# wq2012/SpectralCluster

Hardware: AMD Instinct MI355X
Metric: predict() calls/sec, n=8192 d=256 ICASSP2018 (GraphCut, eigengap k in [2,20], cosine k-means) (higher is better)
Workload: dtype f64; 1 GPU; icassp2018_graphcut_n8192_d256_k8_max20; n_samples=8192, n_features=256, parallelism=replicas x1, collectives=none

## Files before the change

### spectralcluster_amd/csrc/eig.hip

```cpp
#include <algorithm>
#include <cstring>
#include <mutex>

#include "sc_internal.h"

namespace sc {

typedef double v4f64 __attribute__((ext_vector_type(4)));
constexpr int B = kEigBlock;
constexpr int RB = 256 / B;
static_assert(B == 8 || B == 16, "block width must divide the 16-wide MFMA tile");

__device__ __forceinline__ uint64_t splitmix64(uint64_t x) {
  x += 0x9E3779B97F4A7C15ull;
  x = (x ^ (x >> 30)) * 0xBF58476D1CE4E5B9ull;
  x = (x ^ (x >> 27)) * 0x94D049BB133111EBull;
  return x ^ (x >> 31);
}
__device__ __forceinline__ double hash_uniform(uint64_t seed, uint64_t idx) {
  const uint64_t h = splitmix64(seed ^ splitmix64(idx));
  return (double)(h >> 11) * (2.0 / 9007199254740992.0) - 1.0;
}

__global__ void k_random_block(double* W, int n, uint64_t seed) {
  const int e = blockIdx.x * blockDim.x + threadIdx.x;
  if (e < n * B) W[e] = hash_uniform(seed, (uint64_t)e);
}

__global__ void k_refill_deficient(double* W, int n, const int* flags,
                                   uint64_t seed) {
  const int e = blockIdx.x * blockDim.x + threadIdx.x;
  if (e >= n * B) return;
  if ((flags[0] >> (e & (B - 1))) & 1) W[e] = hash_uniform(seed, (uint64_t)e);
}

constexpr int kMvWaves = 8;
__device__ __forceinline__ void block_matvec_body(
    const double* __restrict__ S, int ld, int n, const double* __restrict__ cvec,
    const double* __restrict__ pvec, const double* __restrict__ V, int ldv,
    const double* __restrict__ Vs, double* __restrict__ W) {
  __shared__ double red[kMvWaves][64][4];
  const int lane = threadIdx.x & 63;
  const int wave = threadIdx.x >> 6;
  const int li = lane & 15, lg = lane >> 4;
  const int r0 = blockIdx.x * 16;
  int ri = r0 + li;
  ri = ri < n ? ri : n - 1;
  const double* srow = S + (size_t)ri * ld + 2 * lg;
  v4f64 acc0 = {0.0, 0.0, 0.0, 0.0}, acc1 = {0.0, 0.0, 0.0, 0.0};
  const int nchunks = (n + 31) / 32;
  double2 cur[4], nxt[4];
  auto load = [&](double2* dst, int ch) {
    const int kb = ch * 32 + 2 * lg;
#pragma unroll
    for (int q = 0; q < 4; ++q) {
      if (kb + 8 * q + 1 < ld)
        dst[q] = *reinterpret_cast<const double2*>(srow + ch * 32 + 8 * q);
      else
        dst[q] = make_double2(0.0, 0.0);
    }
  };
  int ch = wave;
  if (ch < nchunks) load(cur, ch);
  for (; ch < nchunks; ch += kMvWaves) {
    if (ch + kMvWaves < nchunks) load(nxt, ch + kMvWaves);
    const int kb = ch * 32 + 2 * lg;
    double b[8];
#pragma unroll
    for (int t = 0; t < 8; ++t) {
      const int k = kb + 8 * (t >> 1) + (t & 1);
      b[t] = (k < n && li < B) ? Vs[(size_t)k * B + li] : 0.0;
    }
#pragma unroll
    for (int q = 0; q < 4; ++q) {
      const double a0 = (kb + 8 * q < n) ? cur[q].x : 0.0;
      const double a1 = (kb + 8 * q + 1 < n) ? cur[q].y : 0.0;
      acc0 = __builtin_amdgcn_mfma_f64_16x16x4f64(a0, b[2 * q], acc0, 0, 0, 0);
      acc1 = __builtin_amdgcn_mfma_f64_16x16x4f64(a1, b[2 * q + 1], acc1, 0, 0, 0);
    }
#pragma unroll
    for (int q = 0; q < 4; ++q) cur[q] = nxt[q];
  }
#pragma unroll
  for (int r = 0; r < 4; ++r) red[wave][lane][r] = acc0[r] + acc1[r];
  __syncthreads();
  if (wave == 0) {
#pragma unroll
    for (int r = 0; r < 4; ++r) {
      double sum = 0.0;
#pragma unroll
      for (int w = 0; w < kMvWaves; ++w) sum += red[w][lane][r];
      const int row = r0 + lg + 4 * r;
      if (row < n && li < B)
        W[(size_t)row * B + li] =
            __builtin_fma(cvec ? cvec[row] : 1.0, sum,
                          pvec ? pvec[row] * V[(size_t)row * ldv + li] : 0.0);
    }
  }
}
__global__ __launch_bounds__(64 * kMvWaves) void k_block_matvec(
    const double* __restrict__ S, int ld, int n, const double* __restrict__ cvec,
    const double* __restrict__ pvec, const double* __restrict__ V, int ldv,
    const double* __restrict__ Vs, double* __restrict__ W) {
  block_matvec_body(S, ld, n, cvec, pvec, V, ldv, Vs, W);
}
__global__ __launch_bounds__(64 * kMvWaves) void k_block_matvec_g(const GroupOf<MatvecItem> g) {
  const MatvecItem& a = g.s[blockIdx.y];
  if ((int)blockIdx.x * 16 >= a.n) return;
  block_matvec_body(a.S, a.ld, a.n, a.cvec, a.pvec, a.V, a.ldv, a.Vs, a.W);
}

constexpr int kSymTile = 128;
constexpr int kSymPitch = 34;
__device__ __forceinline__ int sym_item_id(int I, int J, int nt) {
  return I * nt - I * (I - 1) / 2 + (J - I);
}
__device__ __forceinline__ void block_matvec_sym_body(
    const double* __restrict__ S, int ld, int n, const double* __restrict__ Vs,
    double* __restrict__ pdirect, double* __restrict__ pmirror, int nt) {
  __shared__ __attribute__((aligned(16))) double smem[4 * 32 * kSymPitch];
  int I = 0, rem = blockIdx.x, rowlen = nt;
  while (rem >= rowlen) {
    rem -= rowlen;
    --rowlen;
    ++I;
  }
  const int J = I + rem;
  const bool diag = I == J;
  const int lane = threadIdx.x & 63, wave = threadIdx.x >> 6;
  const int li = lane & 15, lg = lane >> 4;
  const int r0 = I * kSymTile + 32 * wave;
  const int c0 = J * kSymTile;
  double* patch = smem + wave * (32 * kSymPitch);
  double bm[8];
#pragma unroll
  for (int t = 0; t < 8; ++t) {
    const int row = r0 + 4 * t + lg;
    bm[t] = (row < n && li < B) ? Vs[(size_t)row * B + li] : 0.0;
  }
  v4f64 accd[2] = {{0.0, 0.0, 0.0, 0.0}, {0.0, 0.0, 0.0, 0.0}};
  v4f64 accm[4][2];
#pragma unroll
  for (int cs = 0; cs < 4; ++cs)
#pragma unroll
    for (int ct = 0; ct < 2; ++ct) accm[cs][ct] = (v4f64){0.0, 0.0, 0.0, 0.0};
  double2 a[1][2][4];
  auto load = [&](int buf, int cs) {
#pragma unroll
    for (int rt = 0; rt < 2; ++rt) {
      int row = r0 + 16 * rt + li;
      row = row < n ? row : n - 1;
      const double* src = S + (size_t)row * ld + c0 + 32 * cs + 2 * lg;
#pragma unroll
      for (int q = 0; q < 4; ++q) {
        if (c0 + 32 * cs + 8 * q + 2 * lg + 1 < ld)
          a[buf][rt][q] = *reinterpret_cast<const double2*>(src + 8 * q);
        else
          a[buf][rt][q] = make_double2(0.0, 0.0);
      }
    }
  };
#pragma unroll
  for (int cs = 0; cs < 4; ++cs) {
    constexpr int cur = 0;
    load(cur, cs);
    const int kb = c0 + 32 * cs + 2 * lg;
#pragma unroll
    for (int rt = 0; rt < 2; ++rt) {
      const bool rok = r0 + 16 * rt + li < n;
#pragma unroll
      for (int q = 0; q < 4; ++q) {
        if (!rok || kb + 8 * q >= n) a[cur][rt][q].x = 0.0;
        if (!rok || kb + 8 * q + 1 >= n) a[cur][rt][q].y = 0.0;
      }
    }
    double b[8];
#pragma unroll
    for (int t = 0; t < 8; ++t) {
      const int k = kb + 8 * (t >> 1) + (t & 1);
      b[t] = (k < n && li < B) ? Vs[(size_t)k * B + li] : 0.0;
    }
#pragma unroll
    for (int rt = 0; rt < 2; ++rt)
#pragma unroll
      for (int q = 0; q < 4; ++q) {
        accd[rt] = __builtin_amdgcn_mfma_f64_16x16x4f64(a[cur][rt][q].x, b[2 * q], accd[rt], 0, 0, 0);
        accd[rt] = __builtin_amdgcn_mfma_f64_16x16x4f64(a[cur][rt][q].y, b[2 * q + 1], accd[rt], 0, 0, 0);
      }
    if (!diag) {
#pragma unroll
      for (int rt = 0; rt < 2; ++rt)
#pragma unroll
        for (int q = 0; q < 4; ++q)
          *reinterpret_cast<double2*>(patch + (16 * rt + li) * kSymPitch + 8 * q + 2 * lg) =
              a[cur][rt][q];
      __builtin_amdgcn_fence(__ATOMIC_RELEASE, "wavefront");
      __builtin_amdgcn_wave_barrier();
#pragma unroll
      for (int ct = 0; ct < 2; ++ct)
#pragma unroll
        for (int t = 0; t < 8; ++t) {
          const double at = patch[(4 * t + lg) * kSymPitch + 16 * ct + li];
          accm[cs][ct] = __builtin_amdgcn_mfma_f64_16x16x4f64(at, bm[t], accm[cs][ct], 0, 0, 0);
        }
      __builtin_amdgcn_fence(__ATOMIC_ACQUIRE, "wavefront");
      __builtin_amdgcn_wave_barrier();
    }
  }
  const size_t item = blockIdx.x;
  if (li < B) {
#pragma unroll
    for (int rt = 0; rt < 2; ++rt)
#pragma unroll
      for (int r = 0; r < 4; ++r)
        pdirect[(item * kSymTile + 32 * wave + 16 * rt + lg + 4 * r) * B + li] = accd[rt][r];
  }
  if (diag) return;
  __syncthreads();
  double* red = smem;
  if (li < B) {
#pragma unroll
    for (int cs = 0; cs < 4; ++cs)
#pragma unroll
      for (int ct = 0; ct < 2; ++ct)
#pragma unroll
        for (int r = 0; r < 4; ++r)
          red[(wave * kSymTile + 32 * cs + 16 * ct + lg + 4 * r) * B + li] = accm[cs][ct][r];
  }
  __syncthreads();
  for (int e = threadIdx.x; e < kSymTile * B; e += 256)
    pmirror[item * (kSymTile * B) + e] =
        ((red[e] + red[kSymTile * B + e]) + red[2 * kSymTile * B + e]) + red[3 * kSymTile * B + e];
}
__global__ __launch_bounds__(256) void k_block_matvec_sym(
    const double* __restrict__ S, int ld, int n, const double* __restrict__ Vs,
    double* __restrict__ pdirect, double* __restrict__ pmirror, int nt) {
  block_matvec_sym_body(S, ld, n, Vs, pdirect, pmirror, nt);
}
__global__ __launch_bounds__(256) void k_block_matvec_sym_g(const GroupOf<MatvecItem> g) {
  const MatvecItem& a = g.s[blockIdx.y];
  const int nt = (a.n + kSymTile - 1) / kSymTile;
  if ((int)blockIdx.x >= nt * (nt + 1) / 2) return;
  block_matvec_sym_body(a.S, a.ld, a.n, a.Vs, a.slabs, a.slabs + (size_t)(nt * (nt + 1) / 2) * kSymTile * B, nt);
}

__device__ __forceinline__ void matvec_sym_reduce_body(
    const double* __restrict__ pdirect, const double* __restrict__ pmirror, int nt, int n,
    const double* __restrict__ cvec, const double* __restrict__ pvec,
    const double* __restrict__ V, int ldv, double* __restrict__ W) {
  const int R = blockIdx.x / 4;
  const int e = (blockIdx.x & 3) * 256 + threadIdx.x;
  const int rl = e / B, v = e % B;
  const int row = R * kSymTile + rl;
  double acc = 0.0;
  const int total = nt;
  for (int s0 = 0; s0 < total; s0 += 8) {
    double x[8];
#pragma unroll
    for (int u = 0; u < 8; ++u) {
      const int sidx = s0 + u;
      x[u] = 0.0;
      if (sidx < nt - R) {
        x[u] = pdirect[(size_t)sym_item_id(R, R + sidx, nt) * (kSymTile * B) + e];
      } else if (sidx < total) {
        x[u] = pmirror[(size_t)sym_item_id(sidx - (nt - R), R, nt) * (kSymTile * B) + e];
      }
    }
#pragma unroll
    for (int u = 0; u < 8; ++u) acc += x[u];
  }
  if (row < n) W[(size_t)row * B + v] =
      __builtin_fma(cvec ? cvec[row] : 1.0, acc, pvec ? pvec[row] * V[(size_t)row * ldv + v] : 0.0);
}
__global__ __launch_bounds__(256) void k_matvec_sym_reduce(
    const double* __restrict__ pdirect, const double* __restrict__ pmirror, int nt, int n,
    const double* __restrict__ cvec, const double* __restrict__ pvec,
    const double* __restrict__ V, int ldv, double* __restrict__ W) {
  matvec_sym_reduce_body(pdirect, pmirror, nt, n, cvec, pvec, V, ldv, W);
}
__global__ __launch_bounds__(256) void k_matvec_sym_reduce_g(const GroupOf<MatvecItem> g) {
  const MatvecItem& a = g.s[blockIdx.y];
  const int nt = (a.n + kSymTile - 1) / kSymTile;
  if ((int)blockIdx.x >= nt * 4) return;
  matvec_sym_reduce_body(a.slabs, a.slabs + (size_t)(nt * (nt + 1) / 2) * kSymTile * B, nt, a.n,
                         a.cvec, a.pvec, a.V, a.ldv, a.W);
}

constexpr int kProjGroups = 256 / B;
constexpr int kProjAcc = (kLdq + kProjGroups - 1) / kProjGroups;
__global__ __launch_bounds__(256) void k_proj_partial(
    const double* __restrict__ Q, int ldq, int m, const double* __restrict__ W,
    int n, double* __restrict__ partial) {
  __shared__ double Ql[8][kLdq];
  __shared__ double Wl[8][B];
  const int tid = threadIdx.x;
  const int jj = tid % B, ig = tid / B;
  const int rows_per = (n + gridDim.x - 1) / gridDim.x;
  const int rbeg = blockIdx.x * rows_per;
  const int rend = min(n, rbeg + rows_per);
  double acc[kProjAcc];
#pragma unroll
  for (int q = 0; q < kProjAcc; ++q) acc[q] = 0.0;
  for (int r = rbeg; r < rend; r += 8) {
    __syncthreads();
    for (int e = tid; e < 8 * m; e += 256) {
      const int rr = e / m, i = e - rr * m;
      Ql[rr][i] = (r + rr < rend) ? Q[(size_t)(r + rr) * ldq + i] : 0.0;
    }
    if (tid < 8 * B) {
      const int rr = tid / B;
      Wl[rr][jj] = (r + rr < rend) ? W[(size_t)(r + rr) * B + jj] : 0.0;
    }
    __syncthreads();
#pragma unroll
    for (int rr = 0; rr < 8; ++rr) {
      const double w = Wl[rr][jj];
#pragma unroll
      for (int q = 0; q < kProjAcc; ++q)
        if (ig + kProjGroups * q < m)
          acc[q] = __builtin_fma(Ql[rr][ig + kProjGroups * q], w, acc[q]);
    }
  }
  double* out = partial + (size_t)blockIdx.x * (kLdq * B);
#pragma unroll
  for (int q = 0; q < kProjAcc; ++q)
    if (ig + kProjGroups * q < m) out[(ig + kProjGroups * q) * B + jj] = acc[q];
}

__global__ __launch_bounds__(256) void k_reduce_H(
    const double* __restrict__ partial, int nparts, int m, double* __restrict__ Hbuf,
    double* __restrict__ T, int ldt, int col0, int accumulate,
    double* __restrict__ hsq) {
  __shared__ double sq[32];
  const int tid = threadIdx.x;
  const int sub = tid & 7;
  const int e = blockIdx.x * 32 + (tid >> 3);
  double h = 0.0;
  if (e < m * B)
    for (int g = sub; g < nparts; g += 8) h += partial[(size_t)g * (kLdq * B) + e];
  h += __shfl_xor(h, 1);
  h += __shfl_xor(h, 2);
  h += __shfl_xor(h, 4);
  if (sub == 0) {
    if (e < m * B) {
      Hbuf[e] = h;
      if (T != nullptr) {
        const int i = e / B, j = col0 + (e % B);
        if (i <= j) {
          const double v = accumulate ? T[(size_t)i * ldt + j] + h : h;
          T[(size_t)i * ldt + j] = v;
          T[(size_t)j * ldt + i] = v;
        }
      }
    } else {
      h = 0.0;
    }
    sq[tid >> 3] = h * h;
  }
  __syncthreads();
  if (tid < B) {
    double s = 0.0;
    for (int q = tid; q < 32; q += B) s += sq[q];
    atomicAdd(&hsq[tid], s);
  }
}

__global__ __launch_bounds__(256) void k_update_block(
    const double* __restrict__ Q, int ldq, int m, const double* __restrict__ Hbuf,
    double* __restrict__ W, int n) {
  __shared__ double Hl[kLdq * B];
  __shared__ double Ql[RB][kLdq + 1];
  const int tid = threadIdx.x;
  const int jj = tid % B, rr = tid / B;
  const int r0 = blockIdx.x * RB;
  for (int e = tid; e < m * B; e += 256) Hl[e] = Hbuf[e];
  for (int e = tid; e < RB * m; e += 256) {
    const int a = e / m, i = e - a * m;
    Ql[a][i] = (r0 + a < n) ? Q[(size_t)(r0 + a) * ldq + i] : 0.0;
  }
  __syncthreads();
  const int r = r0 + rr;
  if (r < n) {
    double acc = W[(size_t)r * B + jj];
    for (int i = 0; i < m; ++i) acc = __builtin_fma(-Ql[rr][i], Hl[i * B + jj], acc);
    W[(size_t)r * B + jj] = acc;
  }
}

__device__ __forceinline__ void chol8_wave(const double* G, double* __restrict__ Rinv,
                                           const double* __restrict__ hsq,
                                           int* __restrict__ flags,
                                           int* __restrict__ defect_flag, int flag_mode,
                                           int* __restrict__ sticky_flag = nullptr,
                                           int sticky_m = 0, bool sticky_on_defect = true);

__global__ __launch_bounds__(256) void k_reduce_chol(
    const double* __restrict__ partial, int nparts, double* __restrict__ Rinv,
    double* __restrict__ Gsave, const double* __restrict__ hsq,
    int* __restrict__ flags, int* __restrict__ defect_flag, int flag_mode) {
  static_assert(B == 8, "the factorisation below maps the 8 x 8 matrix onto one wavefront");
  __shared__ double G[B * B];
  const int tid = threadIdx.x;
  {
    constexpr int kLanes = 256 / (B * B);
    const int e = tid / kLanes, sub = tid % kLanes;
    double g = 0.0;
    for (int q = sub; q < nparts; q += kLanes) g += partial[(size_t)q * (kLdq * B) + e];
#pragma unroll
    for (int o = 1; o < kLanes; o <<= 1) g += __shfl_xor(g, o);
    if (sub == 0) {
      G[e] = g;
      if (Gsave) Gsave[e] = g;
    }
  }
  __syncthreads();
  if (tid >= 64) return;
  chol8_wave(G, Rinv, hsq, flags, defect_flag, flag_mode);
}

__device__ __forceinline__ void chol8_wave(const double* G, double* __restrict__ Rinv,
                                           const double* __restrict__ hsq,
                                           int* __restrict__ flags,
                                           int* __restrict__ defect_flag, int flag_mode,
                                           int* __restrict__ sticky_flag, int sticky_m,
                                           bool sticky_on_defect) {
// ... 962 lines not shown
```

### spectralcluster_amd/csrc/kmeans_chain.hip

```cpp
#include <algorithm>
#include <cstring>
#include <mutex>

#include "kmeans_common.h"
#include "sc_internal.h"

namespace sc {

constexpr int kKmT = 128;
constexpr int kKmW = kKmT / 64;
constexpr int kKmMaxG = 1024;

struct KmChain {
  const double* ET;
  int lde, n, k, G;
  const double* rnd;
  int trials, first_center, max_iter;
  double* closest;
  double* xsq;
  long long* labels64;
  double* centroids_out;
  double* pm;
  double* meang;
  double* ppot;
  double* pT;
  double* pS[2];
  double* pD[2];
  double* meand;
  double* cent[2];
  int* seeds;
  int* cand[2];
  int* info;
};

__device__ __forceinline__ double km_ordered_sum(const double* src, int stride, int G) {
  double acc = 0.0;
  for (int g0 = 0; g0 < G; g0 += 16) {
    double v[16];
#pragma unroll
    for (int u = 0; u < 16; ++u) v[u] = (g0 + u < G) ? src[(size_t)(g0 + u) * stride] : 0.0;
#pragma unroll
    for (int u = 0; u < 16; ++u) acc += v[u];
  }
  return acc;
}

__device__ __forceinline__ void km_mean(const KmChain& a, double* mean) {
  if ((int)threadIdx.x < a.k) mean[threadIdx.x] = a.meang[threadIdx.x];
}

__device__ __forceinline__ void km_meanreduce_body(const KmChain& a) {
  if ((int)threadIdx.x < a.k)
    a.meang[threadIdx.x] = km_ordered_sum(a.pm + threadIdx.x, 64, a.G) / (double)a.n;
}
__global__ __launch_bounds__(64) void km_meanreduce(const KmChain a) { km_meanreduce_body(a); }
__global__ __launch_bounds__(64) void km_meanreduce_g(const GroupOf<KmChain> g) {
  const KmChain& a = g.s[blockIdx.y];
  if (a.G > 0) km_meanreduce_body(a);
}

template <int KC>
__device__ __forceinline__ void km_load_row(const KmChain& a, int r, double (&v)[KC]) {
#pragma unroll
  for (int j = 0; j < KC; ++j) v[j] = (j < a.k && r < a.n) ? a.ET[(size_t)j * a.lde + r] : 0.0;
}

template <int KC>
__device__ __forceinline__ void km_colsum_body(const KmChain& a) {
  __shared__ double sm[kKmW][KC];
  const int tid = threadIdx.x, r = blockIdx.x * kKmT + tid;
  double v[KC];
  km_load_row<KC>(a, r, v);
#pragma unroll
  for (int j = 0; j < KC; ++j) {
    const double s = wave_sum(v[j]);
    if ((tid & 63) == 0) sm[tid >> 6][j] = s;
  }
  __syncthreads();
  if (tid < a.k) {
    double t = 0.0;
#pragma unroll
    for (int w = 0; w < kKmW; ++w) t += sm[w][tid];
    a.pm[(size_t)blockIdx.x * 64 + tid] = t;
  }
}
template <int KC>
__global__ __launch_bounds__(kKmT) void km_colsum(const KmChain a) {
  km_colsum_body<KC>(a);
}
template <int KC>
__global__ __launch_bounds__(kKmT) void km_colsum_g(const GroupOf<KmChain> g) {
  const KmChain& a = g.s[blockIdx.y];
  if ((int)blockIdx.x >= a.G) return;
  km_colsum_body<KC>(a);
}

template <int KC>
__device__ __forceinline__ double km_dist(const double (&v)[KC], const double* mean,
                                          const double* crow, double csq, double xsq, int k) {
  double dot = 0.0;
#pragma unroll
  for (int j = 0; j < KC; ++j)
    if (j < k) dot += crow[j] * (v[j] - mean[j]);
  double d = -2.0 * dot;
  d += csq;
  d += xsq;
  return fmax(d, 0.0);
}

template <int KC>
__device__ __forceinline__ void km_first_body(const KmChain& a) {
  __shared__ double mean[KC], crow[KC], sm[kKmW];
  __shared__ double csq;
  const int tid = threadIdx.x, r = blockIdx.x * kKmT + tid;
  km_mean(a, mean);
  double v[KC];
  km_load_row<KC>(a, r, v);
  __syncthreads();
  if (tid < a.k) crow[tid] = a.ET[(size_t)tid * a.lde + a.first_center] - mean[tid];
  __syncthreads();
  if (tid == 0) {
    double s2 = 0.0;
    for (int j = 0; j < a.k; ++j) s2 += crow[j] * crow[j];
    csq = s2;
  }
  double xs = 0.0;
#pragma unroll
  for (int j = 0; j < KC; ++j)
    if (j < a.k) {
      const double x = v[j] - mean[j];
      xs += x * x;
    }
  __syncthreads();
  double d = 0.0;
  if (r < a.n) {
    d = km_dist<KC>(v, mean, crow, csq, xs, a.k);
    a.xsq[r] = xs;
    a.closest[r] = d;
  }
  const double tot = block_sum<kKmW>(d, sm);
  if (tid == 0) a.ppot[blockIdx.x] = tot;
  if (blockIdx.x == 0) {
    if (tid == 0) {
      a.seeds[0] = a.first_center;
      a.info[0] = 0;
      a.info[8] = 0;
    }
    if (tid < 8) a.cand[1][tid] = a.n - 1;
  }
}
template <int KC>
__global__ __launch_bounds__(kKmT) void km_first(const KmChain a) {
  km_first_body<KC>(a);
}
template <int KC>
__global__ __launch_bounds__(kKmT) void km_first_g(const GroupOf<KmChain> g) {
  const KmChain& a = g.s[blockIdx.y];
  if ((int)blockIdx.x >= a.G) return;
  km_first_body<KC>(a);
}

__device__ __forceinline__ int km_best_trial(const KmChain& a, double* pots) {
  if ((int)threadIdx.x < a.trials) pots[threadIdx.x] = km_ordered_sum(a.pT + threadIdx.x, 8, a.G);
  __syncthreads();
  int best = 0;
  double bp = pots[0];
  for (int t = 1; t < a.trials; ++t)
    if (pots[t] < bp) {
      bp = pots[t];
      best = t;
    }
  return best;
}

__device__ __forceinline__ void km_prefix(const double* src, int stride, int G, double* part,
                                          double* offset, double* total) {
  for (int g = threadIdx.x; g < G; g += kKmT) part[g] = src[(size_t)g * stride];
  __syncthreads();
  if (threadIdx.x == 0) {
    double off = 0.0, tot = 0.0;
    for (int g = 0; g < G; ++g) {
      if (g == (int)blockIdx.x) off = tot;
      tot += part[g];
    }
    part[kKmMaxG] = off;
    part[kKmMaxG + 1] = tot;
  }
  __syncthreads();
  *offset = part[kKmMaxG];
  *total = part[kKmMaxG + 1];
}

template <int KC>
__device__ __forceinline__ void km_select_body(const KmChain& a, int c) {
  __shared__ double mean[KC], crow[KC], sm[kKmW], pots[8], rvals[8], scan[kKmT];
  __shared__ double part[kKmMaxG + 2];
  __shared__ double csq;
  const int tid = threadIdx.x, lane = tid & 63, wave = tid >> 6;
  const int r = blockIdx.x * kKmT + tid;
  double cl = r < a.n ? a.closest[r] : 0.0;
  double offset = 0.0, pot = 0.0;
  if (c >= 2) {
    km_mean(a, mean);
    double v[KC];
    km_load_row<KC>(a, r, v);
    const double xs = r < a.n ? a.xsq[r] : 0.0;
    __syncthreads();
    const int best = km_best_trial(a, pots);
    const int row = a.cand[(c - 1) & 1][best];
    if (tid < a.k) crow[tid] = a.ET[(size_t)tid * a.lde + row] - mean[tid];
    __syncthreads();
    if (tid == 0) {
      double s2 = 0.0;
      for (int j = 0; j < a.k; ++j) s2 += crow[j] * crow[j];
      csq = s2;
      if (blockIdx.x == 0) a.seeds[c - 1] = row;
    }
    __syncthreads();
    if (r < a.n) {
      cl = fmin(cl, km_dist<KC>(v, mean, crow, csq, xs, a.k));
      a.closest[r] = cl;
    }
    km_prefix(a.pT + best, 8, a.G, part, &offset, &pot);
  } else {
    km_prefix(a.ppot, 1, a.G, part, &offset, &pot);
  }
  if (tid < a.trials) rvals[tid] = a.rnd[(c - 1) * a.trials + tid] * pot;
  double v = cl;
#pragma unroll
  for (int o = 1; o < 64; o <<= 1) {
    const double u = __shfl_up(v, o);
    if (lane >= o) v += u;
  }
  __syncthreads();
  if (lane == 63) sm[wave] = v;
  __syncthreads();
  double woff = 0.0;
  for (int w = 0; w < wave; ++w) woff += sm[w];
  scan[tid] = v + woff;
  __syncthreads();
  if (r < a.n) {
    const double incl = offset + scan[tid];
    const double excl = tid == 0 ? offset : offset + scan[tid - 1];
    for (int t = 0; t < a.trials; ++t) {
      const double rv = rvals[t];
      if ((rv > excl || r == 0) && rv <= incl) atomicMin(&a.cand[c & 1][t], r);
    }
  }
}
template <int KC>
__global__ __launch_bounds__(kKmT) void km_select(const KmChain a, int c) {
  km_select_body<KC>(a, c);
}
template <int KC>
__global__ __launch_bounds__(kKmT) void km_select_g(const GroupOf<KmChain> g, int c) {
  const KmChain& a = g.s[blockIdx.y];
  if ((int)blockIdx.x >= a.G || c >= a.k) return;
  km_select_body<KC>(a, c);
}

template <int KC>
__device__ __forceinline__ void km_trials_body(const KmChain& a, int c) {
  __shared__ double mean[KC], crow[8][KC], csq[8], sm[kKmW];
  const int tid = threadIdx.x, r = blockIdx.x * kKmT + tid;
  km_mean(a, mean);
  double v[KC];
  km_load_row<KC>(a, r, v);
  const double xs = r < a.n ? a.xsq[r] : 0.0;
  const double cl = r < a.n ? a.closest[r] : 0.0;
  __syncthreads();
  for (int e = tid; e < a.trials * a.k; e += kKmT) {
    const int t = e / a.k, j = e - t * a.k;
    crow[t][j] = a.ET[(size_t)j * a.lde + a.cand[c & 1][t]] - mean[j];
  }
  __syncthreads();
  if (tid < a.trials) {
    double s2 = 0.0;
    for (int j = 0; j < a.k; ++j) s2 += crow[tid][j] * crow[tid][j];
    csq[tid] = s2;
  }
  __syncthreads();
  for (int t = 0; t < a.trials; ++t) {
    double d = 0.0;
    if (r < a.n) d = fmin(cl, km_dist<KC>(v, mean, crow[t], csq[t], xs, a.k));
    const double tot = block_sum<kKmW>(d, sm);
    if (tid == 0) a.pT[(size_t)blockIdx.x * 8 + t] = tot;
  }
  if (blockIdx.x == 0 && tid < 8) a.cand[(c + 1) & 1][tid] = a.n - 1;
}
template <int KC>
__global__ __launch_bounds__(kKmT) void km_trials(const KmChain a, int c) {
  km_trials_body<KC>(a, c);
}
template <int KC>
__global__ __launch_bounds__(kKmT) void km_trials_g(const GroupOf<KmChain> g, int c) {
  const KmChain& a = g.s[blockIdx.y];
  if ((int)blockIdx.x >= a.G || c >= a.k) return;
  km_trials_body<KC>(a, c);
}

template <int KC>
__device__ __forceinline__ void km_cluster_partials(const KmChain& a, const double (&v)[KC],
                                                    const double* shift, int label, int r,
                                                    double* vals, int* labs, double* out) {
  const int tid = threadIdx.x, k = a.k;
  labs[tid] = r < a.n ? label : -1;
#pragma unroll
  for (int j = 0; j < KC; ++j)
    if (j < k) vals[tid * KC + j] = v[j] - shift[j];
  __syncthreads();
  const int r0 = blockIdx.x * kKmT;
  const int nsum = k * k + 2 * k;
  for (int base = 0; base < nsum; base += kKmT / 4) {
    const int e = base + (tid >> 2), seg = tid & 3;
    double acc = 0.0;
    if (e < nsum) {
      const int t0 = seg * (kKmT / 4);
      if (e < k * k) {
        const int c2 = e / k, j = e - c2 * k;
#pragma unroll 8
        for (int t = t0; t < t0 + kKmT / 4; ++t) acc += labs[t] == c2 ? vals[t * KC + j] : 0.0;
      } else if (e < k * k + k) {
        const int c2 = e - k * k;
#pragma unroll 8
        for (int t = t0; t < t0 + kKmT / 4; ++t) acc += labs[t] == c2 ? 1.0 : 0.0;
      } else {
        const int c2 = e - k * k - k;
#pragma unroll 8
        for (int t = t0; t < t0 + kKmT / 4; ++t)
          acc += (labs[t] == c2 && r0 + t > 0) ? 1.0 : 0.0;
      }
    }
    const double a1 = __shfl_down(acc, 1), a2 = __shfl_down(acc, 2), a3 = __shfl_down(acc, 3);
    if (e < nsum && seg == 0) out[e] = ((acc + a1) + a2) + a3;
  }
}

template <int KC>
__device__ __forceinline__ void km_lloyd_body(const KmChain& a) {
  extern __shared__ __attribute__((aligned(16))) double dyn[];
  double* vals = dyn;
  int* labs = reinterpret_cast<int*>(vals + kKmT * KC);
  __shared__ double mean[KC], cent[KC * KC], cnorm[KC], pots[8];
  __shared__ int seeds[KC];
  const int tid = threadIdx.x, r = blockIdx.x * kKmT + tid, k = a.k;
  km_mean(a, mean);
  double v[KC];
  km_load_row<KC>(a, r, v);
  __syncthreads();
  if (k > 1) {
    const int best = km_best_trial(a, pots);
    if (tid == 0) {
      seeds[k - 1] = a.cand[(k - 1) & 1][best];
      if (blockIdx.x == 0) a.seeds[k - 1] = seeds[k - 1];
    }
  }
  if (tid < k - 1 || (k == 1 && tid == 0)) seeds[tid] = a.seeds[tid];
  __syncthreads();
  for (int e = tid; e < k * k; e += kKmT) {
    const int c2 = e / k, j = e - c2 * k;
    cent[e] = a.ET[(size_t)j * a.lde + seeds[c2]] - mean[j];
  }
  __syncthreads();
  if (tid < k) {
    double s2 = 0.0;
    for (int j = 0; j < k; ++j) s2 += cent[tid * k + j] * cent[tid * k + j];
    cnorm[tid] = s2;
  }
  __syncthreads();
  int best = 0;
  double bd = INFINITY;
  for (int c2 = 0; c2 < k; ++c2) {
    double dot = 0.0;
#pragma unroll
    for (int j = 0; j < KC; ++j)
      if (j < k) dot += (v[j] - mean[j]) * cent[c2 * k + j];
    const double d = cnorm[c2] - 2.0 * dot;
    if (d < bd) {
      bd = d;
      best = c2;
    }
  }
  km_cluster_partials<KC>(a, v, mean, best, r, vals, labs,
                          a.pS[0] + (size_t)blockIdx.x * (k * k + 2 * k));
}
template <int KC>
__global__ __launch_bounds__(kKmT) void km_lloyd(const KmChain a) {
  km_lloyd_body<KC>(a);
}
template <int KC>
__global__ __launch_bounds__(kKmT) void km_lloyd_g(const GroupOf<KmChain> g) {
  const KmChain& a = g.s[blockIdx.y];
  if ((int)blockIdx.x >= a.G) return;
  km_lloyd_body<KC>(a);
}

template <int KC>
__device__ __forceinline__ void km_cosine_body(const KmChain& a, int it) {
  extern __shared__ __attribute__((aligned(16))) double dyn[];
  double* vals = dyn;
  int* labs = reinterpret_cast<int*>(vals + kKmT * KC);
  __shared__ double mean[KC], cent[KC * KC], cnorm[KC], tot[KC * KC + 2 * KC], sm[kKmW];
  __shared__ double zero[KC];
  __shared__ int seeds[KC];
  __shared__ int s_done;
  const int tid = threadIdx.x, r = blockIdx.x * kKmT + tid, k = a.k;
  if (a.info[8] != 0) return;
  const int nsum = k * k + 2 * k;
  double v[KC];
  km_load_row<KC>(a, r, v);
  if (tid < KC) zero[tid] = 0.0;
  if (it > 0) {
    if (tid == 0) {
      const double mean_d = km_ordered_sum(a.pD[it & 1], 1, a.G) / (double)a.n;
      const double prev = it >= 2 ? a.meand[it - 2] : 0.0;
      s_done = ((mean_d <= prev && mean_d >= (1.0 - 0.001) * prev) || it - 1 == a.max_iter)
                   ? 1 : 0;
      if (blockIdx.x == 0) {
        a.meand[it - 1] = mean_d;
        if (s_done) {
          a.info[0] = it;
          a.info[8] = 1;
        }
      }
    }
    __syncthreads();
    if (s_done) {
      if (blockIdx.x == 0)
        for (int e = tid; e < k * k; e += kKmT)
          a.centroids_out[e] = a.cent[(it - 1) & 1][e];
      return;
    }
  }
  for (int e = tid; e < nsum; e += kKmT) tot[e] = km_ordered_sum(a.pS[it & 1] + e, nsum, a.G);
  if (it == 0) {
    km_mean(a, mean);
    if (tid < k) seeds[tid] = a.seeds[tid];
    __syncthreads();
    for (int e = tid; e < k * k; e += kKmT) {
      const int c2 = e / k, j = e - c2 * k;
      const double count = tot[k * k + c2];
      const double seedv = a.ET[(size_t)j * a.lde + seeds[c2]] - mean[j];
      cent[e] = (count > 0.0 ? tot[e] / count : seedv) + mean[j];
    }
  } else {
    __syncthreads();
    for (int e = tid; e < k * k; e += kKmT) {
      const int c2 = e / k;
      const double count = tot[k * k + c2], nz = tot[k * k + k + c2];
      cent[e] = nz > 0.0 ? tot[e] / count : a.cent[(it - 1) & 1][e];
    }
  }
  __syncthreads();
  if (blockIdx.x == 0)
    for (int e = tid; e < k * k; e += kKmT) a.cent[it & 1][e] = cent[e];
  if (tid < k) {
    double s2 = 0.0;
    for (int j = 0; j < k; ++j) s2 += cent[tid * k + j] * cent[tid * k + j];
    cnorm[tid] = sqrt(s2);
  }
  __syncthreads();
  double en = 0.0;
#pragma unroll
  for (int j = 0; j < KC; ++j)
    if (j < k) en += v[j] * v[j];
  en = sqrt(en);
  int best = 0;
  double bd = INFINITY;
  for (int c2 = 0; c2 < k; ++c2) {
    double dot = 0.0;
#pragma unroll
    for (int j = 0; j < KC; ++j)
      if (j < k) dot += v[j] * cent[c2 * k + j];
    double cosine = dot / (en * cnorm[c2]);
    if (fabs(cosine) > 1.0) cosine = copysign(1.0, cosine);
    const double d = 1.0 - cosine;
    if (d < bd) {
      bd = d;
      best = c2;
    }
  }
  if (r < a.n) a.labels64[r] = best;
  const double dsum = block_sum<kKmW>(r < a.n ? bd : 0.0, sm);
  if (tid == 0) a.pD[(it + 1) & 1][blockIdx.x] = dsum;
  km_cluster_partials<KC>(a, v, zero, best, r, vals, labs,
                          a.pS[(it + 1) & 1] + (size_t)blockIdx.x * nsum);
}
template <int KC>
__global__ __launch_bounds__(kKmT) void km_cosine(const KmChain a, int it) {
  km_cosine_body<KC>(a, it);
}
template <int KC>
__global__ __launch_bounds__(kKmT) void km_cosine_g(const GroupOf<KmChain> g, int it) {
  const KmChain& a = g.s[blockIdx.y];
  if ((int)blockIdx.x >= a.G) return;
  km_cosine_body<KC>(a, it);
}

size_t kmeans_chain_workspace_doubles(int n) {
  const size_t G = (size_t)(n + kKmT - 1) / kKmT;
  return G * 64 + 64 + G + G * 8 + 2 * G * (32 * 32 + 64) + 2 * G + 512 + 2 * 32 * 32 + 256;
}

bool kmeans_chain_supported(int n, int k, int trials) {
  if (k < 1 || k > 32 || trials > 8 || n < 1) return false;
  const size_t G = (size_t)(n + kKmT - 1) / kKmT;
  return G <= (size_t)kKmMaxG && G * (size_t)(k * k + 2 * k) <= 65536;
}

static KmChain km_args(const double* ET, int lde, int n, int k, int max_iter, int first_center,
                       int trials, const KmeansWorkspace& ws) {
  KmChain a;
  a.ET = ET;
  a.lde = lde;
  a.n = n;
  a.k = k;
  a.G = (n + kKmT - 1) / kKmT;
  a.rnd = ws.rnd;
  a.trials = trials;
  a.first_center = first_center;
  a.max_iter = max_iter;
  a.closest = ws.closest;
  a.xsq = ws.xsq;
  a.labels64 = ws.labels64;
  a.centroids_out = ws.centroids;
  const size_t G = a.G;
  double* p = ws.chain;
  a.pm = p;          p += G * 64;
  a.meang = p;       p += 64;
  a.ppot = p;        p += G;
  a.pT = p;          p += G * 8;
  a.pS[0] = p;       p += G * (32 * 32 + 64);
  a.pS[1] = p;       p += G * (32 * 32 + 64);
  a.pD[0] = p;       p += G;
  a.pD[1] = p;       p += G;
  a.meand = p;       p += 512;
  a.cent[0] = p;     p += 32 * 32;
  a.cent[1] = p;     p += 32 * 32;
  int* ip = reinterpret_cast<int*>(p);
  a.seeds = ip;
  a.cand[0] = ip + 64;
  a.cand[1] = ip + 72;
  a.info = ws.info;
  return a;
}

template <int KC>
static void km_enqueue(hipStream_t s, const KmChain& a, int it_begin, int it_count) {
  const dim3 grid(a.G), block(kKmT);
  const size_t dyn = sizeof(double) * kKmT * KC + sizeof(int) * kKmT;
  static std::once_flag once[16];
  int dev = 0;
  hipGetDevice(&dev);
  std::call_once(once[dev & 15], [] {
    hipFuncSetAttribute(reinterpret_cast<const void*>(km_lloyd<KC>),
                        hipFuncAttributeMaxDynamicSharedMemorySize, 96 * 1024);
    hipFuncSetAttribute(reinterpret_cast<const void*>(km_cosine<KC>),
                        hipFuncAttributeMaxDynamicSharedMemorySize, 96 * 1024);
  });
  if (it_begin == 0) {
    hipLaunchKernelGGL(km_colsum<KC>, grid, block, 0, s, a);
    hipLaunchKernelGGL(km_meanreduce, dim3(1), dim3(64), 0, s, a);
    hipLaunchKernelGGL(km_first<KC>, grid, block, 0, s, a);
    for (int c = 1; c < a.k; ++c) {
      hipLaunchKernelGGL(km_select<KC>, grid, block, 0, s, a, c);
      hipLaunchKernelGGL(km_trials<KC>, grid, block, 0, s, a, c);
    }
    hipLaunchKernelGGL(km_lloyd<KC>, grid, block, dyn, s, a);
  }
  for (int it = it_begin; it < it_begin + it_count; ++it)
    hipLaunchKernelGGL(km_cosine<KC>, grid, block, dyn, s, a, it);
}

template <int KC>
static void km_enqueue_group(hipStream_t s, const GroupOf<KmChain>& g, int count, int gmax,
                             int kmax, int it_begin, int it_count) {
  const dim3 grid(gmax, count), block(kKmT);
  const size_t dyn = sizeof(double) * kKmT * KC + sizeof(int) * kKmT;
  SC_OPT_IN_LDS(km_lloyd_g<KC>, 96 * 1024);
  SC_OPT_IN_LDS(km_cosine_g<KC>, 96 * 1024);
  if (it_begin == 0) {
    hipLaunchKernelGGL(km_colsum_g<KC>, grid, block, 0, s, g);
    hipLaunchKernelGGL(km_meanreduce_g, dim3(1, count), dim3(64), 0, s, g);
    hipLaunchKernelGGL(km_first_g<KC>, grid, block, 0, s, g);
    for (int c = 1; c < kmax; ++c) {
      hipLaunchKernelGGL(km_select_g<KC>, grid, block, 0, s, g, c);
      hipLaunchKernelGGL(km_trials_g<KC>, grid, block, 0, s, g, c);
    }
    hipLaunchKernelGGL(km_lloyd_g<KC>, grid, block, dyn, s, g);
  }
  for (int it = it_begin; it < it_begin + it_count; ++it)
    hipLaunchKernelGGL(km_cosine_g<KC>, grid, block, dyn, s, g, it);
}

void launch_kmeans_chain_group(hipStream_t s, const KmGroupItem* items, int count, int it_begin,
                               int it_count) {
  GroupOf<KmChain> g;
  memset(&g, 0, sizeof(g));
  int gmax = 0, kmax = 0;
  for (int z = 0; z < count; ++z) {
    const KmGroupItem& it = items[z];
    if (it.n <= 0) continue;
    g.s[z] = km_args(it.ET, it.lde, it.n, it.k, it.max_iter, it.first_center, it.trials, it.ws);
    gmax = std::max(gmax, g.s[z].G);
    kmax = std::max(kmax, it.k);
  }
  if (gmax == 0) return;
  if (kmax <= 8) km_enqueue_group<8>(s, g, count, gmax, kmax, it_begin, it_count);
  else if (kmax <= 16) km_enqueue_group<16>(s, g, count, gmax, kmax, it_begin, it_count);
  else km_enqueue_group<32>(s, g, count, gmax, kmax, it_begin, it_count);
}

void launch_kmeans_chain(hipStream_t s, const double* ET, int lde, int n, int k, int max_iter,
                         int first_center, int trials, const KmeansWorkspace& ws, int it_begin,
                         int it_count) {
  const KmChain a = km_args(ET, lde, n, k, max_iter, first_center, trials, ws);
  if (k <= 8) km_enqueue<8>(s, a, it_begin, it_count);
  else if (k <= 16) km_enqueue<16>(s, a, it_begin, it_count);
  else km_enqueue<32>(s, a, it_begin, it_count);
}

}
```

Before: 390.6 calls/s.

## Batch ordered-sum loads and fold k-means mean/seed lookups into chain kernels

Adds a shared ordered_sum helper that issues 64 strided loads before a sched barrier and then adds them in fixed order. This is meant to hide memory latency in the serial partial-sum reductions of the eigen matvec and k-means chain. The k-means chain also drops the separate mean-reduce kernel, folding it into km_first. It stores centered candidate/centroid rows and their norms in a workspace so later kernels stop doing dependent seed-index ET gathers, and it hoists independent loads ahead of barriers. The cost is redundant per-block reductions and heavier register use from 64-wide load arrays.

After: 393.3 calls/s (median of 3 runs). No clear change (+0.7%).

```diff
diff --git a/spectralcluster_amd/csrc/eig.hip b/spectralcluster_amd/csrc/eig.hip
--- a/spectralcluster_amd/csrc/eig.hip
+++ b/spectralcluster_amd/csrc/eig.hip
@@ -2,6 +2,7 @@
 #include <cstring>
 #include <mutex>
 
+#include "ordered_sum.h"
 #include "sc_internal.h"
 
 namespace sc {
@@ -252,25 +253,16 @@
   const int e = (blockIdx.x & 3) * 256 + threadIdx.x;
   const int rl = e / B, v = e % B;
   const int row = R * kSymTile + rl;
-  double acc = 0.0;
-  const int total = nt;
-  for (int s0 = 0; s0 < total; s0 += 8) {
-    double x[8];
-#pragma unroll
-    for (int u = 0; u < 8; ++u) {
-      const int sidx = s0 + u;
-      x[u] = 0.0;
-      if (sidx < nt - R) {
-        x[u] = pdirect[(size_t)sym_item_id(R, R + sidx, nt) * (kSymTile * B) + e];
-      } else if (sidx < total) {
-        x[u] = pmirror[(size_t)sym_item_id(sidx - (nt - R), R, nt) * (kSymTile * B) + e];
-      }
-    }
-#pragma unroll
-    for (int u = 0; u < 8; ++u) acc += x[u];
-  }
-  if (row < n) W[(size_t)row * B + v] =
-      __builtin_fma(cvec ? cvec[row] : 1.0, acc, pvec ? pvec[row] * V[(size_t)row * ldv + v] : 0.0);
+  const int rc = row < n ? row : n - 1;
+  const double cr = cvec ? cvec[rc] : 1.0;
+  const double pr = pvec ? pvec[rc] : 0.0;
+  const double vr = pvec ? V[(size_t)rc * ldv + v] : 0.0;
+  const int ndirect = nt - R;
+  const double acc = ordered_sum_at(nt, [=](int sidx) {
+    const int id = sidx < ndirect ? sym_item_id(R, R + sidx, nt) : sym_item_id(sidx - ndirect, R, nt);
+    return (sidx < ndirect ? pdirect : pmirror) + (size_t)id * (kSymTile * B) + e;
+  });
+  if (row < n) W[(size_t)row * B + v] = __builtin_fma(cr, acc, pvec ? pr * vr : 0.0);
 }
 __global__ __launch_bounds__(256) void k_matvec_sym_reduce(
     const double* __restrict__ pdirect, const double* __restrict__ pmirror, int nt, int n,
diff --git a/spectralcluster_amd/csrc/kmeans_chain.hip b/spectralcluster_amd/csrc/kmeans_chain.hip
--- a/spectralcluster_amd/csrc/kmeans_chain.hip
+++ b/spectralcluster_amd/csrc/kmeans_chain.hip
@@ -3,6 +3,7 @@
 #include <mutex>
 
 #include "kmeans_common.h"
+#include "ordered_sum.h"
 #include "sc_internal.h"
 
 namespace sc {
@@ -28,36 +29,20 @@
   double* pD[2];
   double* meand;
   double* cent[2];
-  int* seeds;
+  double* rows;
   int* cand[2];
   int* info;
 };
 
-__device__ __forceinline__ double km_ordered_sum(const double* src, int stride, int G) {
-  double acc = 0.0;
-  for (int g0 = 0; g0 < G; g0 += 16) {
-    double v[16];
-#pragma unroll
-    for (int u = 0; u < 16; ++u) v[u] = (g0 + u < G) ? src[(size_t)(g0 + u) * stride] : 0.0;
-#pragma unroll
-    for (int u = 0; u < 16; ++u) acc += v[u];
-  }
-  return acc;
-}
-
-__device__ __forceinline__ void km_mean(const KmChain& a, double* mean) {
-  if ((int)threadIdx.x < a.k) mean[threadIdx.x] = a.meang[threadIdx.x];
-}
-
-__device__ __forceinline__ void km_meanreduce_body(const KmChain& a) {
-  if ((int)threadIdx.x < a.k)
-    a.meang[threadIdx.x] = km_ordered_sum(a.pm + threadIdx.x, 64, a.G) / (double)a.n;
-}
-__global__ __launch_bounds__(64) void km_meanreduce(const KmChain a) { km_meanreduce_body(a); }
-__global__ __launch_bounds__(64) void km_meanreduce_g(const GroupOf<KmChain> g) {
-  const KmChain& a = g.s[blockIdx.y];
-  if (a.G > 0) km_meanreduce_body(a);
-}
+__device__ __forceinline__ int km_opaque_zero() {
+  int z = 0;
+  asm volatile("" : "+v"(z));
+  return z;
+}
+
+constexpr int kKmCsq = 256;
+constexpr int kKmCent = 264;
+
 
 template <int KC>
 __device__ __forceinline__ void km_load_row(const KmChain& a, int r, double (&v)[KC]) {
@@ -113,11 +98,18 @@
   __shared__ double mean[KC], crow[KC], sm[kKmW];
   __shared__ double csq;
   const int tid = threadIdx.x, r = blockIdx.x * kKmT + tid;
-  km_mean(a, mean);
   double v[KC];
   km_load_row<KC>(a, r, v);
-  __syncthreads();
-  if (tid < a.k) crow[tid] = a.ET[(size_t)tid * a.lde + a.first_center] - mean[tid];
+  if (tid < a.k) {
+    const double first = a.ET[(size_t)tid * a.lde + a.first_center];
+    const double mu = ordered_sum(a.pm + tid, 64, a.G) / (double)a.n;
+    mean[tid] = mu;
+    crow[tid] = first - mu;
+    if (blockIdx.x == 0) {
+      a.meang[tid] = mu;
+      a.rows[kKmCent + tid] = first - mu;
+    }
+  }
   __syncthreads();
   if (tid == 0) {
     double s2 = 0.0;
@@ -142,7 +134,6 @@
   if (tid == 0) a.ppot[blockIdx.x] = tot;
   if (blockIdx.x == 0) {
     if (tid == 0) {
-      a.seeds[0] = a.first_center;
       a.info[0] = 0;
       a.info[8] = 0;
     }
@@ -160,12 +151,10 @@
   km_first_body<KC>(a);
 }
 
-__device__ __forceinline__ int km_best_trial(const KmChain& a, double* pots) {
-  if ((int)threadIdx.x < a.trials) pots[threadIdx.x] = km_ordered_sum(a.pT + threadIdx.x, 8, a.G);
-  __syncthreads();
+__device__ __forceinline__ int km_argmin(const double* pots, int trials) {
   int best = 0;
   double bp = pots[0];
-  for (int t = 1; t < a.trials; ++t)
+  for (int t = 1; t < trials; ++t)
     if (pots[t] < bp) {
       bp = pots[t];
       best = t;
@@ -173,78 +162,69 @@
   return best;
 }
 
-__device__ __forceinline__ void km_prefix(const double* src, int stride, int G, double* part,
-                                          double* offset, double* total) {
-  for (int g = threadIdx.x; g < G; g += kKmT) part[g] = src[(size_t)g * stride];
-  __syncthreads();
-  if (threadIdx.x == 0) {
-    double off = 0.0, tot = 0.0;
-    for (int g = 0; g < G; ++g) {
-      if (g == (int)blockIdx.x) off = tot;
-      tot += part[g];
-    }
-    part[kKmMaxG] = off;
-    part[kKmMaxG + 1] = tot;
-  }
-  __syncthreads();
-  *offset = part[kKmMaxG];
-  *total = part[kKmMaxG + 1];
-}
-
 template <int KC>
 __device__ __forceinline__ void km_select_body(const KmChain& a, int c) {
-  __shared__ double mean[KC], crow[KC], sm[kKmW], pots[8], rvals[8], scan[kKmT];
-  __shared__ double part[kKmMaxG + 2];
-  __shared__ double csq;
+  __shared__ double mean[KC], sm[kKmW], pots[8], offs[8], rvals[8], scan[kKmT];
+  __shared__ double tc[8 * KC], tcs[8];
   const int tid = threadIdx.x, lane = tid & 63, wave = tid >> 6;
-  const int r = blockIdx.x * kKmT + tid;
+  const int r = blockIdx.x * kKmT + tid, k = a.k;
   double cl = r < a.n ? a.closest[r] : 0.0;
-  double offset = 0.0, pot = 0.0;
+  const double rv = tid < a.trials ? a.rnd[(c - 1) * a.trials + tid] : 0.0;
+  double v[KC];
+  double xs = 0.0, mu = 0.0, tcv[2] = {0.0, 0.0}, tq = 0.0;
   if (c >= 2) {
-    km_mean(a, mean);
-    double v[KC];
     km_load_row<KC>(a, r, v);
-    const double xs = r < a.n ? a.xsq[r] : 0.0;
-    __syncthreads();
-    const int best = km_best_trial(a, pots);
-    const int row = a.cand[(c - 1) & 1][best];
-    if (tid < a.k) crow[tid] = a.ET[(size_t)tid * a.lde + row] - mean[tid];
-    __syncthreads();
-    if (tid == 0) {
-      double s2 = 0.0;
-      for (int j = 0; j < a.k; ++j) s2 += crow[j] * crow[j];
-      csq = s2;
-      if (blockIdx.x == 0) a.seeds[c - 1] = row;
-    }
-    __syncthreads();
+    if (r < a.n) xs = a.xsq[r];
+    if (tid < k) mu = a.meang[tid];
+#pragma unroll
+    for (int u = 0; u < 2; ++u) tcv[u] = a.rows[tid + u * kKmT];
+    if (tid < a.trials) tq = a.rows[kKmCsq + tid];
+  }
+  const int nt = c >= 2 ? a.trials : 1;
+  double tot = 0.0, off = 0.0;
+  if (tid < nt)
+    tot = ordered_sum_split(c >= 2 ? a.pT + tid : a.ppot, c >= 2 ? 8 : 1, a.G, blockIdx.x, &off);
+  if (tid < nt) {
+    pots[tid] = tot;
+    offs[tid] = off;
+  }
+  if (c >= 2) {
+    if (tid < k) mean[tid] = mu;
+#pragma unroll
+    for (int u = 0; u < 2; ++u)
+      if (tid + u * kKmT < a.trials * k) tc[tid + u * kKmT] = tcv[u];
+    if (tid < a.trials) tcs[tid] = tq;
+  }
+  __syncthreads();
+  const int best = km_argmin(pots, nt);
+  const double offset = offs[best], pot = pots[best];
+  if (c >= 2) {
     if (r < a.n) {
-      cl = fmin(cl, km_dist<KC>(v, mean, crow, csq, xs, a.k));
+      cl = fmin(cl, km_dist<KC>(v, mean, tc + best * k, tcs[best], xs, k));
       a.closest[r] = cl;
     }
-    km_prefix(a.pT + best, 8, a.G, part, &offset, &pot);
-  } else {
-    km_prefix(a.ppot, 1, a.G, part, &offset, &pot);
-  }
-  if (tid < a.trials) rvals[tid] = a.rnd[(c - 1) * a.trials + tid] * pot;
-  double v = cl;
+    if (blockIdx.x == 0 && tid < k) a.rows[kKmCent + (c - 1) * 32 + tid] = tc[best * k + tid];
+  }
+  if (tid < a.trials) rvals[tid] = rv * pot;
+  double sv = cl;
 #pragma unroll
   for (int o = 1; o < 64; o <<= 1) {
-    const double u = __shfl_up(v, o);
-    if (lane >= o) v += u;
-  }
-  __syncthreads();
-  if (lane == 63) sm[wave] = v;
+    const double u = __shfl_up(sv, o);
+    if (lane >= o) sv += u;
+  }
+  __syncthreads();
+  if (lane == 63) sm[wave] = sv;
   __syncthreads();
   double woff = 0.0;
   for (int w = 0; w < wave; ++w) woff += sm[w];
-  scan[tid] = v + woff;
+  scan[tid] = sv + woff;
   __syncthreads();
   if (r < a.n) {
     const double incl = offset + scan[tid];
     const double excl = tid == 0 ? offset : offset + scan[tid - 1];
     for (int t = 0; t < a.trials; ++t) {
-      const double rv = rvals[t];
-      if ((rv > excl || r == 0) && rv <= incl) atomicMin(&a.cand[c & 1][t], r);
+      const double rvt = rvals[t];
+      if ((rvt > excl || r == 0) && rvt <= incl) atomicMin(&a.cand[c & 1][t], r);
     }
   }
 }
@@ -262,27 +242,43 @@
 template <int KC>
 __device__ __forceinline__ void km_trials_body(const KmChain& a, int c) {
   __shared__ double mean[KC], crow[8][KC], csq[8], sm[kKmW];
-  const int tid = threadIdx.x, r = blockIdx.x * kKmT + tid;
-  km_mean(a, mean);
+  __shared__ int rows[8];
+  const int tid = threadIdx.x, r = blockIdx.x * kKmT + tid, k = a.k;
   double v[KC];
   km_load_row<KC>(a, r, v);
   const double xs = r < a.n ? a.xsq[r] : 0.0;
   const double cl = r < a.n ? a.closest[r] : 0.0;
-  __syncthreads();
-  for (int e = tid; e < a.trials * a.k; e += kKmT) {
-    const int t = e / a.k, j = e - t * a.k;
-    crow[t][j] = a.ET[(size_t)j * a.lde + a.cand[c & 1][t]] - mean[j];
+  const double mu = tid < k ? a.meang[tid] : 0.0;
+  const int cd = tid < a.trials ? a.cand[c & 1][tid] : 0;
+  if (tid < k) mean[tid] = mu;
+  if (tid < a.trials) rows[tid] = cd;
+  __syncthreads();
+  double cv[2] = {0.0, 0.0};
+#pragma unroll
+  for (int u = 0; u < 2; ++u) {
+    const int e = tid + u * kKmT, ec = e < a.trials * k ? e : a.trials * k - 1;
+    cv[u] = a.ET[(size_t)(ec % k) * a.lde + rows[ec / k]];
+  }
+#pragma unroll
+  for (int u = 0; u < 2; ++u) {
+    const int e = tid + u * kKmT;
+    if (e < a.trials * k) {
+      const double x = cv[u] - mean[e % k];
+      crow[e / k][e % k] = x;
+      if (blockIdx.x == 0) a.rows[e] = x;
+    }
   }
   __syncthreads();
   if (tid < a.trials) {
     double s2 = 0.0;
-    for (int j = 0; j < a.k; ++j) s2 += crow[tid][j] * crow[tid][j];
+    for (int j = 0; j < k; ++j) s2 += crow[tid][j] * crow[tid][j];
     csq[tid] = s2;
+    if (blockIdx.x == 0) a.rows[kKmCsq + tid] = s2;
   }
   __syncthreads();
   for (int t = 0; t < a.trials; ++t) {
     double d = 0.0;
-    if (r < a.n) d = fmin(cl, km_dist<KC>(v, mean, crow[t], csq[t], xs, a.k));
+    if (r < a.n) d = fmin(cl, km_dist<KC>(v, mean, crow[t], csq[t], xs, k));
     const double tot = block_sum<kKmW>(d, sm);
     if (tid == 0) a.pT[(size_t)blockIdx.x * 8 + t] = tot;
   }
@@ -341,25 +337,40 @@
   extern __shared__ __attribute__((aligned(16))) double dyn[];
   double* vals = dyn;
   int* labs = reinterpret_cast<int*>(vals + kKmT * KC);
-  __shared__ double mean[KC], cent[KC * KC], cnorm[KC], pots[8];
-  __shared__ int seeds[KC];
+  constexpr int kPer = (KC * KC + kKmT - 1) / kKmT;
+  __shared__ double mean[KC], cent[KC * KC], cnorm[KC], pots[8], tc[8 * KC];
   const int tid = threadIdx.x, r = blockIdx.x * kKmT + tid, k = a.k;
-  km_mean(a, mean);
   double v[KC];
   km_load_row<KC>(a, r, v);
-  __syncthreads();
+  const double mu = tid < k ? a.meang[tid] : 0.0;
+  const int nold = k > 1 ? (k - 1) * k : k * k;
+  double cv[kPer], tcv[2] = {0.0, 0.0};
+#pragma unroll
+  for (int u = 0; u < kPer; ++u) {
+    const int e = tid + u * kKmT;
+    cv[u] = e < nold ? a.rows[kKmCent + (e / k) * 32 + e % k] : 0.0;
+  }
+  double pot = 0.0;
   if (k > 1) {
-    const int best = km_best_trial(a, pots);
-    if (tid == 0) {
-      seeds[k - 1] = a.cand[(k - 1) & 1][best];
-      if (blockIdx.x == 0) a.seeds[k - 1] = seeds[k - 1];
-    }
-  }
-  if (tid < k - 1 || (k == 1 && tid == 0)) seeds[tid] = a.seeds[tid];
-  __syncthreads();
-  for (int e = tid; e < k * k; e += kKmT) {
-    const int c2 = e / k, j = e - c2 * k;
-    cent[e] = a.ET[(size_t)j * a.lde + seeds[c2]] - mean[j];
+#pragma unroll
+    for (int u = 0; u < 2; ++u) tcv[u] = a.rows[tid + u * kKmT];
+    if (tid < a.trials) pot = ordered_sum(a.pT + tid, 8, a.G);
+    if (tid < a.trials) pots[tid] = pot;
+#pragma unroll
+    for (int u = 0; u < 2; ++u)
+      if (tid + u * kKmT < a.trials * k) tc[tid + u * kKmT] = tcv[u];
+  }
+  if (tid < k) mean[tid] = mu;
+#pragma unroll
+  for (int u = 0; u < kPer; ++u) {
+    const int e = tid + u * kKmT;
+    if (e < nold) cent[e] = cv[u];
+  }
+  __syncthreads();
+  if (k > 1 && tid < k) {
+    const double x = tc[km_argmin(pots, a.trials) * k + tid];
+    cent[(k - 1) * k + tid] = x;
+    if (blockIdx.x == 0) a.rows[kKmCent + (k - 1) * 32 + tid] = x;
   }
   __syncthreads();
   if (tid < k) {
@@ -400,55 +411,67 @@
   extern __shared__ __attribute__((aligned(16))) double dyn[];
   double* vals = dyn;
   int* labs = reinterpret_cast<int*>(vals + kKmT * KC);
-  __shared__ double mean[KC], cent[KC * KC], cnorm[KC], tot[KC * KC + 2 * KC], sm[kKmW];
+  constexpr int kPer = (KC * KC + kKmT - 1) / kKmT;
+  __shared__ double mean[KC], cent[KC * KC], cnorm[KC], tot[KC * KC + 2 * KC + 1], sm[kKmW];
   __shared__ double zero[KC];
-  __shared__ int seeds[KC];
-  __shared__ int s_done;
   const int tid = threadIdx.x, r = blockIdx.x * kKmT + tid, k = a.k;
+  const int nsum = k * k + 2 * k;
   if (a.info[8] != 0) return;
-  const int nsum = k * k + 2 * k;
+  const int z = km_opaque_zero();
   double v[KC];
   km_load_row<KC>(a, r, v);
+  const double prev = it >= 2 ? a.meand[it - 2 + z] : 0.0;
+  const double mu = (it == 0 && tid < k) ? a.meang[tid] : 0.0;
+  double pc[kPer];
+#pragma unroll
+  for (int u = 0; u < kPer; ++u) {
+    const int e = tid + u * kKmT;
+    pc[u] = 0.0;
+    if (e < k * k)
+      pc[u] = it == 0 ? a.rows[kKmCent + (e / k) * 32 + e % k] : a.cent[(it - 1) & 1][e];
+  }
+  const int nent = nsum + (it > 0 ? 1 : 0);
+  for (int base = 0; base < nent; base += kKmT) {
+    const int e = base + tid, ec = e < nent ? e : nent - 1;
+    const double sum = ordered_sum(ec < nsum ? a.pS[it & 1] + ec : a.pD[it & 1],
+                                   ec < nsum ? nsum : 1, a.G);
+    if (e < nent) tot[e] = sum;
+  }
   if (tid < KC) zero[tid] = 0.0;
+  if (it == 0 && tid < k) mean[tid] = mu;
+  __syncthreads();
   if (it > 0) {
-    if (tid == 0) {
-      const double mean_d = km_ordered_sum(a.pD[it & 1], 1, a.G) / (double)a.n;
-      const double prev = it >= 2 ? a.meand[it - 2] : 0.0;
-      s_done = ((mean_d <= prev && mean_d >= (1.0 - 0.001) * prev) || it - 1 == a.max_iter)
-                   ? 1 : 0;
+    const double mean_d = tot[nsum] / (double)a.n;
+    const bool done =
+        (mean_d <= prev && mean_d >= (1.0 - 0.001) * prev) || it - 1 == a.max_iter;
+    if (blockIdx.x == 0 && tid == 0) {
+      a.meand[it - 1] = mean_d;
+      if (done) {
+        a.info[0] = it;
+        a.info[8] = 1;
+      }
+    }
+    if (done) {
       if (blockIdx.x == 0) {
-        a.meand[it - 1] = mean_d;
-        if (s_done) {
-          a.info[0] = it;
-          a.info[8] = 1;
-        }
+#pragma unroll
+        for (int u = 0; u < kPer; ++u)
+          if (tid + u * kKmT < k * k) a.centroids_out[tid + u * kKmT] = pc[u];
       }
-    }
-    __syncthreads();
-    if (s_done) {
-      if (blockIdx.x == 0)
-        for (int e = tid; e < k * k; e += kKmT)
-          a.centroids_out[e] = a.cent[(it - 1) & 1][e];
       return;
     }
   }
-  for (int e = tid; e < nsum; e += kKmT) tot[e] = km_ordered_sum(a.pS[it & 1] + e, nsum, a.G);
-  if (it == 0) {
-    km_mean(a, mean);
-    if (tid < k) seeds[tid] = a.seeds[tid];
-    __syncthreads();
-    for (int e = tid; e < k * k; e += kKmT) {
+#pragma unroll
+  for (int u = 0; u < kPer; ++u) {
+    const int e = tid + u * kKmT;
+    if (e < k * k) {
       const int c2 = e / k, j = e - c2 * k;
       const double count = tot[k * k + c2];
-      const double seedv = a.ET[(size_t)j * a.lde + seeds[c2]] - mean[j];
-      cent[e] = (count > 0.0 ? tot[e] / count : seedv) + mean[j];
-    }
-  } else {
-    __syncthreads();
-    for (int e = tid; e < k * k; e += kKmT) {
-      const int c2 = e / k;
-      const double count = tot[k * k + c2], nz = tot[k * k + k + c2];
-      cent[e] = nz > 0.0 ? tot[e] / count : a.cent[(it - 1) & 1][e];
+      if (it == 0) {
+        cent[e] = (count > 0.0 ? tot[e] / count : pc[u]) + mean[j];
+      } else {
+        const double nz = tot[k * k + k + c2];
+        cent[e] = nz > 0.0 ? tot[e] / count : pc[u];
+      }
     }
   }
   __syncthreads();
@@ -499,7 +522,8 @@
 
 size_t kmeans_chain_workspace_doubles(int n) {
   const size_t G = (size_t)(n + kKmT - 1) / kKmT;
-  return G * 64 + 64 + G + G * 8 + 2 * G * (32 * 32 + 64) + 2 * G + 512 + 2 * 32 * 32 + 256;
+  return G * 64 + 64 + G + G * 8 + 2 * G * (32 * 32 + 64) + 2 * G + 512 + 2 * 32 * 32 +
+         (kKmCent + 32 * 32) + 256;
 }
 
 bool kmeans_chain_supported(int n, int k, int trials) {
@@ -537,8 +561,8 @@
   a.meand = p;       p += 512;
   a.cent[0] = p;     p += 32 * 32;
   a.cent[1] = p;     p += 32 * 32;
+  a.rows = p;        p += kKmCent + 32 * 32;
   int* ip = reinterpret_cast<int*>(p);
-  a.seeds = ip;
   a.cand[0] = ip + 64;
   a.cand[1] = ip + 72;
   a.info = ws.info;
@@ -560,7 +584,6 @@
   });
   if (it_begin == 0) {
     hipLaunchKernelGGL(km_colsum<KC>, grid, block, 0, s, a);
-    hipLaunchKernelGGL(km_meanreduce, dim3(1), dim3(64), 0, s, a);
     hipLaunchKernelGGL(km_first<KC>, grid, block, 0, s, a);
     for (int c = 1; c < a.k; ++c) {
       hipLaunchKernelGGL(km_select<KC>, grid, block, 0, s, a, c);
@@ -581,7 +604,6 @@
   SC_OPT_IN_LDS(km_cosine_g<KC>, 96 * 1024);
   if (it_begin == 0) {
     hipLaunchKernelGGL(km_colsum_g<KC>, grid, block, 0, s, g);
-    hipLaunchKernelGGL(km_meanreduce_g, dim3(1, count), dim3(64), 0, s, g);
     hipLaunchKernelGGL(km_first_g<KC>, grid, block, 0, s, g);
     for (int c = 1; c < kmax; ++c) {
       hipLaunchKernelGGL(km_select_g<KC>, grid, block, 0, s, g, c);
diff --git a/spectralcluster_amd/csrc/ordered_sum.h b/spectralcluster_amd/csrc/ordered_sum.h
--- /dev/null
+++ b/spectralcluster_amd/csrc/ordered_sum.h
@@ -0,0 +1,73 @@
+#ifndef SPECTRALCLUSTER_AMD_ORDERED_SUM_H_
+#define SPECTRALCLUSTER_AMD_ORDERED_SUM_H_
+
+#include <cstddef>
+
+#if defined(__HIPCC__)
+#include <hip/hip_runtime.h>
+#define SC_HD __host__ __device__
+#else
+#define SC_HD
+#endif
+#if defined(__HIP_DEVICE_COMPILE__)
+#define SC_LOADS_BEFORE_ADDS() __builtin_amdgcn_sched_barrier(0)
+#else
+#define SC_LOADS_BEFORE_ADDS() ((void)0)
+#endif
+
+namespace sc {
+
+constexpr int kOrderedSumRound = 64;
+
+template <typename At>
+SC_HD inline double ordered_sum_split_at(int nparts, At at, int split, double* prefix) {
+  double acc = 0.0;
+  for (int p0 = 0; p0 < nparts; p0 += kOrderedSumRound) {
+    const int last = nparts - 1;
+    double v[kOrderedSumRound];
+#pragma unroll
+    for (int u = 0; u < kOrderedSumRound; ++u) v[u] = *at(p0 + u < last ? p0 + u : last);
+    SC_LOADS_BEFORE_ADDS();
+#pragma unroll
+    for (int u = 0; u < kOrderedSumRound; ++u) {
+      if (p0 + u == split) *prefix = acc;
+      acc = (p0 + u <= last) ? acc + v[u] : acc;
+    }
+  }
+  return acc;
+}
+template <typename At>
+SC_HD inline double ordered_sum_at(int nparts, At at) {
+  double unused = 0.0;
+  return ordered_sum_split_at(nparts, at, -1, &unused);
+}
+
+SC_HD inline double ordered_sum_split(const double* src, size_t stride, int nparts, int split,
+                                      double* prefix) {
+  double acc = 0.0;
+  for (int p0 = 0; p0 < nparts; p0 += kOrderedSumRound) {
+    const int left = nparts - 1 - p0;
+    const double* ptr = src + (size_t)p0 * stride;
+    double v[kOrderedSumRound];
+#pragma unroll
+    for (int u = 0; u < kOrderedSumRound; ++u) {
+      v[u] = *ptr;
+      ptr += u < left ? stride : 0;
+    }
+    SC_LOADS_BEFORE_ADDS();
+#pragma unroll
+    for (int u = 0; u < kOrderedSumRound; ++u) {
+      if (p0 + u == split) *prefix = acc;
+      acc = (u <= left) ? acc + v[u] : acc;
+    }
+  }
+  return acc;
+}
+SC_HD inline double ordered_sum(const double* src, size_t stride, int nparts) {
+  double unused = 0.0;
+  return ordered_sum_split(src, stride, nparts, -1, &unused);
+}
+
+}
+
+#endif
```
